# architsharma97/earl_benchmark

Measured on AMD Instinct MI355X. Metric: env steps/sec (aggregate) at N parallel envs, higher is better.
Workload: dtype f64

## Files before the change

### earl_benchmark_amd/csrc/tabletop_rollout_ws.h

```cpp
#pragma once
#include <type_traits>

#include "tabletop_device.h"

#ifndef EARL_WSM_OFF
#define EARL_WSM_OFF 0
#endif

#if !defined(EARL_WS_NO_SMALL_NT) && !defined(EARL_WS_SMALL_NT)
#define EARL_WS_SMALL_NT 1
#endif
#if !defined(EARL_WS_NO_XCD_REMAP) && !defined(EARL_WS_XCD_REMAP)
#define EARL_WS_XCD_REMAP 1
#endif
namespace earl {

typedef int ws_v4i __attribute__((ext_vector_type(4)));
typedef float ws_v4f __attribute__((ext_vector_type(4)));
__device__ __forceinline__ __amdgpu_buffer_rsrc_t ws_rsrc(const void* p) {
  return __builtin_amdgcn_make_buffer_rsrc(const_cast<void*>(p), 0, -1, 0x00020000);
}

struct WsArgs {
  int32_t n, T, horizon, wide;
  const float* __restrict__ act;
  double* __restrict__ qpos;
  int8_t* __restrict__ attached;
  const int32_t* __restrict__ goal_idx;
  const double* __restrict__ goal_table;
  int32_t* __restrict__ steps_since_reset;
  float* __restrict__ obs;
  float* __restrict__ reward;
  uint8_t* __restrict__ done;
  uint8_t* __restrict__ success;
  Thresholds th;
  float grip_x;
  int32_t reset_first;
  earl_tabletop_cfg cfg;
  int32_t* __restrict__ goal_idx_w;
  int32_t* __restrict__ num_interventions;
  int32_t episodes, Tep;
  long long act_ep_stride;
  int32_t wgs, ep_groups, ep_per_group;
};

__device__ __forceinline__ uint64_t ws_ep_counter(const WsArgs& a, int ep) { return a.cfg.counter + (uint64_t)ep * (uint64_t)(a.Tep + 1); }
__device__ __forceinline__ int ws_goal_row_ep(const WsArgs& a, int env, int ep) {
  if (a.reset_first) return sample_goal(a.cfg, ws_ep_counter(a, ep), env, nullptr);
  return a.goal_idx[env];
}

__device__ __forceinline__ int ws_goal_row(const WsArgs& a, int env) {
  if (a.reset_first) return sample_goal(a.cfg, a.cfg.counter, env, nullptr);
  return a.goal_idx[env];
}

__device__ __forceinline__ void wave_lds_fence() {
  __builtin_amdgcn_fence(__ATOMIC_RELEASE, "wavefront");
  __builtin_amdgcn_wave_barrier();
  __builtin_amdgcn_fence(__ATOMIC_ACQUIRE, "wavefront");
}

__device__ __forceinline__ double clip_fast(double x) { return fmin(fmax(x, -2.8), 2.8); }

template <bool EXACT>
__device__ __forceinline__ void ws_step(double& fx, double& fy, double& ox, double& oy, double& oxl, double& oyl,
                                        bool& att, double a0, double a1, bool grip, const Thresholds& th) {
  if constexpr (EXACT) {
    const double dx = fx - ox, dy = fy - oy;
    const bool near = fma(dy, dy, dx * dx) < th.grasp_d2;
    att = grip && (att || near);
    const double nfx = clipd(fx + a0, -2.8, 2.8), nfy = clipd(fy + a1, -2.8, 2.8);
    if (att) {
      ox = clipd(ox + (nfx - fx), -2.8, 2.8);
      oy = clipd(oy + (nfy - fy), -2.8, 2.8);
    }
    fx = nfx;
    fy = nfy;
    oxl = ox;
    oyl = oy;
  } else {
    const double dx = fx - oxl, dy = fy - oyl;
    const bool near = fma(dy, dy, dx * dx) < th.grasp_d2;
    att = grip && (att || near);
    oxl = ox;
    oyl = oy;
    const double nfx = clip_fast(fx + a0), nfy = clip_fast(fy + a1);
    const double ddx = att ? nfx - fx : -0.0, ddy = att ? nfy - fy : -0.0;
    ox = clip_fast(ox + ddx);
    oy = clip_fast(oy + ddy);
    fx = nfx;
    fy = nfy;
  }
}

struct WsConst { double lo, hi, thr; int nz; };
__device__ __forceinline__ void ws_step_v(double& fx, double& fy, double& ox, double& oy, double& oxl, double& oyl,
                                          int& att, double a0, double a1, int grip, const WsConst& k) {
  const double dx = fx - oxl, dy = fy - oyl;
  const int near = __double2hiint(fma(dy, dy, dx * dx) - k.thr) >> 31;
  att = grip & (att | near);
  oxl = ox;
  oyl = oy;
  const double nfx = fmin(fmax(fx + a0, k.lo), k.hi), nfy = fmin(fmax(fy + a1, k.lo), k.hi);
  const double ddx = nfx - fx, ddy = nfy - fy;
  const double sx = __hiloint2double((att & __double2hiint(ddx)) | (~att & k.nz), att & __double2loint(ddx));
  const double sy = __hiloint2double((att & __double2hiint(ddy)) | (~att & k.nz), att & __double2loint(ddy));
  ox = fmin(fmax(ox + sx, k.lo), k.hi);
  oy = fmin(fmax(oy + sy, k.lo), k.hi);
  fx = nfx;
  fy = nfy;
}

__device__ __forceinline__ double both_halves_from_lower(double v) {
  const unsigned lo = __double2loint(v), hi = __double2hiint(v);
  const auto r0 = __builtin_amdgcn_permlane32_swap(lo, lo, false, false);
  const auto r1 = __builtin_amdgcn_permlane32_swap(hi, hi, false, false);
  return __hiloint2double(r1[0], r0[0]);
}
template <bool EXACT>
__device__ __forceinline__ void ws_step_xy(double& f, double& o, double& ol, unsigned long long& att64, double a,
                                           unsigned long long grip64, const Thresholds& th) {
  const double d = f - (EXACT ? o : ol);
  const double d2 = fma(d, d, both_halves_from_lower(d * d));
  const unsigned near_y = (unsigned)(__ballot(d2 < th.grasp_d2) >> 32);
  const unsigned long long near64 = ((unsigned long long)near_y << 32) | near_y;
  att64 = grip64 & (att64 | near64);
  const bool att = __builtin_amdgcn_inverse_ballot_w64(att64);
  if constexpr (EXACT) {
    const double nf = clipd(f + a, -2.8, 2.8);
    if (att) o = clipd(o + (nf - f), -2.8, 2.8);
    f = nf;
    ol = o;
  } else {
    ol = o;
    const double nf = clip_fast(f + a);
    const double dd = att ? nf - f : -0.0;
    o = clip_fast(o + dd);
    f = nf;
  }
}

__device__ __forceinline__ unsigned long long ws_near_mask_xy(double f, double o, const Thresholds& th) {
  const double d = f - o;
  const double d2 = fma(d, d, both_halves_from_lower(d * d));
  const unsigned near_y = (unsigned)(__ballot(d2 < th.grasp_d2) >> 32);
  return ((unsigned long long)near_y << 32) | near_y;
}
__device__ __forceinline__ void ws_step_xy_pipe(double& f, double& o, unsigned long long& nm, unsigned long long& att64,
                                                double a, unsigned long long grip64, const Thresholds& th) {
  att64 = grip64 & (att64 | nm);
  const bool att = __builtin_amdgcn_inverse_ballot_w64(att64);
  const double nf = clip_fast(f + a);
  nm = ws_near_mask_xy(nf, o, th);
  const double dd = att ? nf - f : -0.0;
  o = clip_fast(o + dd);
  f = nf;
}

__device__ __forceinline__ double dpp_from_x(double v) {
  const int lo = __builtin_amdgcn_update_dpp(__double2loint(v), __double2loint(v), 0xA0, 0xF, 0xF, false);
  const int hi = __builtin_amdgcn_update_dpp(__double2hiint(v), __double2hiint(v), 0xA0, 0xF, 0xF, false);
  return __hiloint2double(hi, lo);
}
__device__ __forceinline__ double dpp_swap_pair(double v) {
  const int lo = __builtin_amdgcn_update_dpp(__double2loint(v), __double2loint(v), 0xB1, 0xF, 0xF, false);
  const int hi = __builtin_amdgcn_update_dpp(__double2hiint(v), __double2hiint(v), 0xB1, 0xF, 0xF, false);
  return __hiloint2double(hi, lo);
}
__device__ __forceinline__ int ws_near_mask_adj(double f, double o, const WsConst& k) {
  const double d = f - o;
  const double d2 = fma(d, d, dpp_from_x(d * d));
  const int m = __double2hiint(d2 - k.thr) >> 31;
  return __builtin_amdgcn_update_dpp(m, m, 0xF5, 0xF, 0xF, false);
}
__device__ __forceinline__ void ws_step_adj(double& f, double& o, int& nm, int& attm, double a, int grip, const WsConst& k) {
  attm = grip & (attm | nm);
  const double nf = fmin(fmax(f + a, k.lo), k.hi);
  nm = ws_near_mask_adj(nf, o, k);
  const double dd = nf - f;
  const double sd = __hiloint2double((attm & __double2hiint(dd)) | (~attm & k.nz), attm & __double2loint(dd));
  o = fmin(fmax(o + sd, k.lo), k.hi);
  f = nf;
}
__device__ __forceinline__ void ws_step_adj_exact(double& f, double& o, int& attm, double a, int grip, int c, const Thresholds& th) {
  const double pf = dpp_swap_pair(f), po = dpp_swap_pair(o), pa = dpp_swap_pair(a);
  double fx = c ? pf : f, fy = c ? f : pf, ox = c ? po : o, oy = c ? o : po, oxl = 0, oyl = 0;
  bool att = attm != 0;
  ws_step<true>(fx, fy, ox, oy, oxl, oyl, att, c ? pa : a, c ? a : pa, grip != 0, th);
  f = c ? fy : fx;
  o = c ? oy : ox;
  attm = att ? -1 : 0;
}

__device__ unsigned long long g_ws_prof[64 * 16];
__device__ __forceinline__ unsigned long long ws_clock() {
  unsigned long long t;
  asm volatile("s_memtime %0\n\ts_waitcnt lgkmcnt(0)" : "=s"(t)::"memory");
  return t;
}
#define WS_STAMP(acc)                                  \
  if constexpr (PROF) {                                \
    const unsigned long long t_ = ws_clock();          \
    acc += t_ - p_x;                                   \
    p_x = t_;                                          \
  }

template <int RT, int NC, int NL, int NS, int K, int LEAD, bool PROF = false, bool MULTI = false, bool LDNT = false>
__global__ __launch_bounds__(64 * ((NC == 3 ? 2 : NC) + NL + NS)) void rollout_ws_kernel(const WsArgs a_in) {
  constexpr int E = 64;
  WsArgs a = a_in;
#ifdef EARL_WS_XCD_REMAP
  const int bid = (gridDim.x % 8 == 0) ? (int)((blockIdx.x % 8) * (gridDim.x / 8) + blockIdx.x / 8) : (int)blockIdx.x;
#else
  const int bid = (int)blockIdx.x;
#endif
  int wg = bid;
  bool leaves_state = true;
  int eps_before = 0;
  if constexpr (MULTI) {
    if (a_in.ep_groups > 1) {
      const int grp = bid / a_in.wgs;
      wg = bid - grp * a_in.wgs;
      eps_before = grp * a_in.ep_per_group;
      const int ne = min(a_in.ep_per_group, a_in.episodes - eps_before);
      leaves_state = eps_before + ne == a_in.episodes;
      a.episodes = ne;
      a.T = ne * a_in.Tep;
      a.cfg.counter = a_in.cfg.counter + (uint64_t)eps_before * (uint64_t)(a_in.Tep + 1);
      const size_t row0 = (size_t)eps_before * (size_t)a_in.Tep * (size_t)a_in.n;
      a.act = a_in.act + (size_t)eps_before * (size_t)a_in.act_ep_stride;
      a.obs = a_in.obs + row0 * 12; a.reward = a_in.reward + row0; a.done = a_in.done + row0; a.success = a_in.success + row0;
    }
  }
  constexpr int NCW = NC == 3 ? 2 : NC;
  constexpr int KL = K / NL;
  static_assert(K % NL == 0, "K must be a multiple of NL");
  static_assert(!MULTI || NC == 3, "several episodes per launch: adjacent-lane compute waves only");
  static_assert(NC == 1 || NC == 2 || NC == 3, "NC is 1, 2 or 3");
  __shared__ double A[3][K][2 * E];
  __shared__ uint8_t G[3][K][E];
  __shared__ int slow_flag[3][NL];
  __shared__ float4 R[2][K][E * 3];
  constexpr int SQ = K >= 8 ? 1 : KL;
  __shared__ float S[NL][SQ][E * 3];

  const int wave = __builtin_amdgcn_readfirstlane(threadIdx.x >> 6), lane = threadIdx.x & 63;
  const int n = a.n, T = a.T;
  const int i0 = wg * E;
  const int i = i0 + lane;
  const int valid = min(E, n - i0);
  const bool live = lane < valid;
  const int nch = (T + K - 1) / K;
  unsigned long long p_x = 0, p_t0 = 0;

  if (wave < NCW || wave >= NCW + NL) {
    const int tid = wave < NCW ? (int)threadIdx.x : (int)threadIdx.x - 64 * NL;
    const int e = tid % E;
    float g[6] = {0, 0, 0, 0, 0, 0};
    if (e < valid) load_goal<1>(a.goal_table, ws_goal_row(a, i0 + e), g);
    for (int rowi = tid / E; rowi < 2 * K; rowi += NCW + NS) {
      float4* row = &R[0][0][0] + (size_t)rowi * (E * 3) + e * 3;
      row[1] = float4{-1.0f, -1.0f, g[0], g[1]};
      row[2] = float4{g[2], g[3], g[4], g[5]};
    }
  }

  if (wave < NCW) {
   __builtin_amdgcn_s_setprio(3);
   if constexpr (NC == 3) {
    const int h = lane & 1, el = lane >> 1, e = wave * 32 + el;
    const int ie = i0 + e;
    const bool alive = e < valid;
    double f = 0, o = 0;
    bool att0 = false;
    if (alive) {
      if (a.reset_first) {
        Env<1> ev;
        const int gi = reset_env<1>(ev, a.cfg, a.cfg.counter, ie, a.goal_table, nullptr, a.th);
        f = h ? ev.q[1] : ev.q[0];
        o = h ? ev.q[3] : ev.q[2];
        if (h == 0 && leaves_state) {
          a.goal_idx_w[ie] = gi;
          a.num_interventions[ie] += 1 + eps_before;
        }
      } else {
        f = a.qpos[(size_t)ie * 4 + h];
        o = a.qpos[(size_t)ie * 4 + 2 + h];
        att0 = a.attached[ie] >= 0;
      }
    }
    int attm = att0 ? -1 : 0;
    WsConst kc{-2.8, 2.8, a.th.grasp_d2, (int)0x80000000};
    asm volatile("" : "+v"(kc.lo), "+v"(kc.hi), "+v"(kc.thr), "+v"(kc.nz));
    int nm = ws_near_mask_adj(f, o, kc);
    bool slow = __any(!(fabs(f) <= 1e300) || !(fabs(o) <= 2.8));
    unsigned long long p_read = 0, p_comp = 0, p_bar = 0;
    if constexpr (PROF) p_t0 = ws_clock();
    __syncthreads();
    if constexpr (PROF) p_x = ws_clock();
    const unsigned long long p_first = p_x - p_t0;
    double av[K], nv[K];
    int gv[K], ng[K];
    int nslow = 0;
    auto fetch = [&](int c) {
      const int ab = c % 3;
      nslow = 0;
#pragma unroll
      for (int w = 0; w < NL; ++w) nslow |= slow_flag[ab][w];
#pragma unroll
      for (int k = 0; k < K; ++k) {
        nv[k] = A[ab][k][wave * 64 + lane];
        ng[k] = reinterpret_cast<const int8_t*>(&G[ab][k][0])[e];
      }
    };
    fetch(0);
    constexpr int GR = 8, GPC = K / GR;
    static_assert(!MULTI || (K % GR == 0 && GPC <= 2), "multi-episode launches: chunks of one or two 8-step granules");
    const int gpe = MULTI ? a.Tep / GR : 0x7fffffff;
    int next_ep_g = gpe, ep = 0, last_gi = -1;
    double f_pend = 0, o_pend = 0;
    bool pend = false;
    auto prepare_episode = [&](const int gidx) -> bool {
      if (MULTI && !(EARL_WSM_OFF & 4) && gidx == next_ep_g && gidx * GR < T) {
        ++ep;
        next_ep_g += gpe;
        Env<1> ev;
        last_gi = reset_env<1>(ev, a.cfg, ws_ep_counter(a, ep), ie, a.goal_table, nullptr, a.th);
        f_pend = h ? ev.q[1] : ev.q[0];
        o_pend = h ? ev.q[3] : ev.q[2];
        return true;
      }
      return false;
    };
    auto apply_episode = [&]() {
      f = f_pend; o = o_pend;
      attm = 0;
      nm = ws_near_mask_adj(f, o, kc);
    };
    for (int c = 0; c < nch; ++c) {
      const int rb = c & 1;
      if (prepare_episode(c * (MULTI ? GPC : 1))) apply_episode();
      if constexpr (MULTI && GPC == 2) pend = prepare_episode(c * GPC + 1);
      slow = slow || (nslow != 0);
#pragma unroll
      for (int k = 0; k < K; ++k) { av[k] = nv[k]; gv[k] = ng[k]; }
      if (c + 1 < nch) fetch(c + 1);
      if constexpr (PROF) asm volatile("s_waitcnt lgkmcnt(0)" ::: "memory");
      WS_STAMP(p_read)
      auto run = [&](auto exact, auto full) {
#pragma unroll
        for (int k = 0; k < K; ++k) {
          if constexpr (!decltype(full)::value)
            if (c * K + k >= T) break;
          if constexpr (MULTI && GPC == 2) { if (k == GR && pend) apply_episode(); }
          if constexpr (decltype(exact)::value) ws_step_adj_exact(f, o, attm, av[k], gv[k], h, a.th);
          else ws_step_adj(f, o, nm, attm, av[k], gv[k], kc);
          float* rowf = reinterpret_cast<float*>(&R[rb][k][e * 3]);
          rowf[h] = (float)f;
          rowf[2 + h] = (float)o;
          rowf[4 + h] = __int_as_float(~attm & (int)0xBF800000);
        }
      };
      const bool whole = (c + 1) * K <= T;
      if (__builtin_amdgcn_readfirstlane(slow ? 1 : 0)) {
        if (whole) run(std::true_type{}, std::true_type{}); else run(std::true_type{}, std::false_type{});
      } else {
        if (whole) run(std::false_type{}, std::true_type{}); else run(std::false_type{}, std::false_type{});
      }
      if constexpr (PROF) asm volatile("s_waitcnt lgkmcnt(0)" ::: "memory");
      WS_STAMP(p_comp)
      __syncthreads();
      WS_STAMP(p_bar)
    }
    if constexpr (PROF) {
      if (lane == 0 && bid < 64 && wave == 0) {
        unsigned long long* op = g_ws_prof + bid * 16;
        op[0] = p_first; op[1] = p_read; op[2] = p_comp; op[3] = p_bar; op[4] = p_x - p_t0;
      }
      if (lane == 0 && bid < 64 && wave == 1) g_ws_prof[bid * 16 + 13] = p_bar;
    }
    if (alive && leaves_state) {
      a.qpos[(size_t)ie * 4 + h] = f;
      a.qpos[(size_t)ie * 4 + 2 + h] = o;
      if (h == 0) {
        a.attached[ie] = attm ? 0 : -1;
        a.steps_since_reset[ie] = (a.reset_first ? 0 : a.steps_since_reset[ie]) + (MULTI ? a.Tep : T);
        if (MULTI && ep > 0) {
          a.goal_idx_w[ie] = last_gi;
          a.num_interventions[ie] += ep;
        }
      }
    }
   } else if constexpr (NC == 2) {
    const int h = lane >> 5, el = lane & 31, e = wave * 32 + el;
    const int ie = i0 + e;
    const bool alive = e < valid;
    double f = 0, o = 0;
    bool att0 = false;
    if (alive) {
      if (a.reset_first) {
        Env<1> ev;
        const int gi = reset_env<1>(ev, a.cfg, a.cfg.counter, ie, a.goal_table, nullptr, a.th);
        f = h ? ev.q[1] : ev.q[0];
        o = h ? ev.q[3] : ev.q[2];
        if (h == 0) {
          a.goal_idx_w[ie] = gi;
          a.num_interventions[ie] += 1;
        }
      } else {
        f = a.qpos[(size_t)ie * 4 + h];
        o = a.qpos[(size_t)ie * 4 + 2 + h];
        att0 = a.attached[ie] >= 0;
      }
    }
    double ol = o;
    unsigned long long att64 = __ballot(att0);
    unsigned long long nm = ws_near_mask_xy(f, o, a.th);
    bool slow = __any(!(fabs(f) <= 1e300) || !(fabs(o) <= 2.8));
    unsigned long long p_read = 0, p_comp = 0, p_bar = 0;
    if constexpr (PROF) p_t0 = ws_clock();
    __syncthreads();
    if constexpr (PROF) p_x = ws_clock();
    const unsigned long long p_first = p_x - p_t0;
    double av[K], nv[K];
    uint8_t gv[K], ng[K];
    int nslow = 0;
    auto fetch = [&](int c) {
      const int ab = c % 3;
      nslow = 0;
#pragma unroll
      for (int w = 0; w < NL; ++w) nslow |= slow_flag[ab][w];
#pragma unroll
      for (int k = 0; k < K; ++k) { nv[k] = A[ab][k][wave * 64 + lane]; ng[k] = G[ab][k][e]; }
    };
    fetch(0);
    for (int c = 0; c < nch; ++c) {
      const int rb = c & 1;
      slow = slow || (nslow != 0);
#pragma unroll
      for (int k = 0; k < K; ++k) { av[k] = nv[k]; gv[k] = ng[k]; }
      if (c + 1 < nch) fetch(c + 1);
      if constexpr (PROF) asm volatile("s_waitcnt lgkmcnt(0)" ::: "memory");
      WS_STAMP(p_read)
      auto run = [&](auto exact, auto full) {
#pragma unroll
        for (int k = 0; k < K; ++k) {
          if constexpr (!decltype(full)::value)
            if (c * K + k >= T) break;
          if constexpr (decltype(exact)::value) ws_step_xy<true>(f, o, ol, att64, av[k], __ballot(gv[k] != 0), a.th);
          else ws_step_xy_pipe(f, o, nm, att64, av[k], __ballot(gv[k] != 0), a.th);
          float* rowf = reinterpret_cast<float*>(&R[rb][k][e * 3]);
          rowf[h] = (float)f;
          rowf[2 + h] = (float)o;
          rowf[4 + h] = __builtin_amdgcn_inverse_ballot_w64(att64) ? 0.0f : -1.0f;
        }
      };
      const bool whole = (c + 1) * K <= T;
      if (__builtin_amdgcn_readfirstlane(slow ? 1 : 0)) {
        if (whole) run(std::true_type{}, std::true_type{}); else run(std::true_type{}, std::false_type{});
      } else {
        if (whole) run(std::false_type{}, std::true_type{}); else run(std::false_type{}, std::false_type{});
      }
      if constexpr (PROF) asm volatile("s_waitcnt lgkmcnt(0)" ::: "memory");
      WS_STAMP(p_comp)
      __syncthreads();
      WS_STAMP(p_bar)
    }
    if constexpr (PROF) {
      if (lane == 0 && bid < 64 && wave == 0) {
        unsigned long long* op = g_ws_prof + bid * 16;
        op[0] = p_first; op[1] = p_read; op[2] = p_comp; op[3] = p_bar; op[4] = p_x - p_t0;
      }
    }
    if (alive) {
      a.qpos[(size_t)ie * 4 + h] = f;
      a.qpos[(size_t)ie * 4 + 2 + h] = o;
      if (h == 0) {
        a.attached[ie] = (att64 >> lane) & 1 ? 0 : -1;
        a.steps_since_reset[ie] = (a.reset_first ? 0 : a.steps_since_reset[ie]) + T;
      }
    }
   } else {
    double fx = 0, fy = 0, ox = 0, oy = 0;
    bool att = false;
    if (live) {
      if (a.reset_first) {
        Env<1> ev;
        const int gi = reset_env<1>(ev, a.cfg, a.cfg.counter, i, a.goal_table, nullptr, a.th);
        fx = ev.q[0]; fy = ev.q[1]; ox = ev.q[2]; oy = ev.q[3];
        a.goal_idx_w[i] = gi;
        a.num_interventions[i] += 1;
      } else {
        const double2* q2 = reinterpret_cast<const double2*>(a.qpos + (size_t)i * 4);
        const double2 u = q2[0], v = q2[1];
        fx = u.x; fy = u.y; ox = v.x; oy = v.y;
        att = a.attached[i] >= 0;
      }
    }
    double oxl = ox, oyl = oy;
    int attm = att ? -1 : 0;
    WsConst kc{-2.8, 2.8, a.th.grasp_d2, (int)0x80000000};
    asm volatile("" : "+v"(kc.lo), "+v"(kc.hi), "+v"(kc.thr), "+v"(kc.nz));
    bool slow = __any(!(fabs(fx) <= 1e300) || !(fabs(fy) <= 1e300) || !(fabs(ox) <= 2.8) || !(fabs(oy) <= 2.8));
    unsigned long long p_read = 0, p_comp = 0, p_bar = 0;
    if constexpr (PROF) p_t0 = ws_clock();
    __syncthreads();
    if constexpr (PROF) p_x = ws_clock();
    const unsigned long long p_first = p_x - p_t0;
    double2 av[K], nv[K];
    int gv[K], ng[K];
    int nslow = 0;
    auto fetch = [&](int c) {
      const int ab = c % 3;
      nslow = 0;
#pragma unroll
      for (int w = 0; w < NL; ++w) nslow |= slow_flag[ab][w];
#pragma unroll
      for (int k = 0; k < K; ++k) {
        nv[k] = reinterpret_cast<const double2*>(&A[ab][k][0])[lane];
        ng[k] = reinterpret_cast<const int8_t*>(&G[ab][k][0])[lane];
      }
    };
    fetch(0);
    for (int c = 0; c < nch; ++c) {
      const int rb = c & 1;
      slow = slow || (nslow != 0);
#pragma unroll
      for (int k = 0; k < K; ++k) { av[k] = nv[k]; gv[k] = ng[k]; }
      if (c + 1 < nch) fetch(c + 1);
      if constexpr (PROF) asm volatile("s_waitcnt lgkmcnt(0)" ::: "memory");
      WS_STAMP(p_read)
      auto run = [&](auto exact, auto full) {
#pragma unroll
        for (int k = 0; k < K; ++k) {
          if constexpr (!decltype(full)::value)
            if (c * K + k >= T) break;
          if constexpr (decltype(exact)::value) {
            bool attb = attm != 0;
            ws_step<true>(fx, fy, ox, oy, oxl, oyl, attb, av[k].x, av[k].y, gv[k] != 0, a.th);
            attm = attb ? -1 : 0;
          } else {
            ws_step_v(fx, fy, ox, oy, oxl, oyl, attm, av[k].x, av[k].y, gv[k], kc);
          }
          float4* row = &R[rb][k][lane * 3];
          row[0] = float4{(float)fx, (float)fy, (float)ox, (float)oy};
          const float flag = __int_as_float(~attm & (int)0xBF800000);
          *reinterpret_cast<float2*>(&row[1]) = float2{flag, flag};
        }
      };
      const bool whole = (c + 1) * K <= T;
      if (__builtin_amdgcn_readfirstlane(slow ? 1 : 0)) {
        if (whole) run(std::true_type{}, std::true_type{}); else run(std::true_type{}, std::false_type{});
      } else {
        if (whole) run(std::false_type{}, std::true_type{}); else run(std::false_type{}, std::false_type{});
      }
      if constexpr (PROF) asm volatile("s_waitcnt lgkmcnt(0)" ::: "memory");
      WS_STAMP(p_comp)
      __syncthreads();
      WS_STAMP(p_bar)
    }
    if constexpr (PROF) {
      if (lane == 0 && bid < 64) {
        unsigned long long* o = g_ws_prof + bid * 16;
        o[0] = p_first; o[1] = p_read; o[2] = p_comp; o[3] = p_bar; o[4] = p_x - p_t0;
      }
    }
    if (live) {
      double2* q2 = reinterpret_cast<double2*>(a.qpos + (size_t)i * 4);
      q2[0] = double2{fx, fy};
      q2[1] = double2{ox, oy};
      a.attached[i] = attm ? 0 : -1;
      a.steps_since_reset[i] = (a.reset_first ? 0 : a.steps_since_reset[i]) + T;
    }
   }
  } else if (wave < NCW + NL) {
    const int w = wave - NCW;
    float rawA[LEAD][KL][3], rawB[LEAD][KL][3];
    const int last = max(valid * 3 - 1, 0);
    const int e0 = min(lane, last), e1 = min(lane + 64, last), e2 = min(lane + 128, last);
    const float* const base = a.act + (size_t)i0 * 3;
    const size_t step_stride = (size_t)n * 3;
    constexpr int GR = 8, GPC = MULTI ? K / GR : 1;
    const int gpe = MULTI ? a.Tep / GR : 0x7fffffff;
    int l_ep_end = gpe, l_ep_first = 0;
    size_t l_ep_base = 0;
    auto issue_trip = [&](float (&raw)[LEAD][KL][3], int r) {
      const float* rowp[LEAD][GPC];
      size_t off[LEAD][KL];
#pragma unroll
      for (int d = 0; d < LEAD; ++d) {
        if constexpr (MULTI && !(EARL_WSM_OFF & 1)) {
          const int j = min(r * LEAD + d, nch - 1);
#pragma unroll
          for (int hg = 0; hg < GPC; ++hg) {
            const int gidx = min(j * GPC + hg, T / GR - 1);
            const int xm = -(int)(gidx >= l_ep_end);
            l_ep_end += gpe & xm; l_ep_first += gpe & xm;
            l_ep_base += (size_t)a.act_ep_stride & (size_t)(long long)xm;
            rowp[d][hg] = base + l_ep_base + (size_t)__builtin_amdgcn_readfirstlane((gidx - l_ep_first) * GR + w) * step_stride;
          }
        } else {
#pragma unroll
          for (int q = 0; q < KL; ++q)
            off[d][q] = (size_t)__builtin_amdgcn_readfirstlane(min((r * LEAD + d) * K + q * NL + w, (MULTI ? a.Tep : T) - 1)) * step_stride;
        }
      }
      const size_t qstride = (size_t)NL * step_stride;
      static_assert(!MULTI || GR % NL == 0, "a loader's steps of a granule: a whole number");
      constexpr int QG = MULTI ? GR / NL : KL;
#pragma unroll
      for (int d = 0; d < LEAD; ++d) {
#pragma unroll
        for (int q = 0; q < KL; ++q) {
          const float* p;
          if constexpr (MULTI && !(EARL_WSM_OFF & 1)) p = rowp[d][q / QG] + (size_t)(q % QG) * qstride;
          else p = base + off[d][q];
#ifdef EARL_WS_LD_AUX
          if constexpr (true) {
            const __amdgpu_buffer_rsrc_t rs = ws_rsrc(p);
            raw[d][q][0] = __builtin_bit_cast(float, __builtin_amdgcn_raw_buffer_load_b32(rs, e0 * 4, 0, EARL_WS_LD_AUX));
            raw[d][q][1] = __builtin_bit_cast(float, __builtin_amdgcn_raw_buffer_load_b32(rs, e1 * 4, 0, EARL_WS_LD_AUX));
            raw[d][q][2] = __builtin_bit_cast(float, __builtin_amdgcn_raw_buffer_load_b32(rs, e2 * 4, 0, EARL_WS_LD_AUX));
          } else
#endif
          if constexpr (LDNT) {
            raw[d][q][0] = __builtin_nontemporal_load(p + e0); raw[d][q][1] = __builtin_nontemporal_load(p + e1); raw[d][q][2] = __builtin_nontemporal_load(p + e2);
          } else {
            raw[d][q][0] = p[e0]; raw[d][q][1] = p[e1]; raw[d][q][2] = p[e2];
          }
        }
      }
    };
    unsigned long long p_proc = 0, p_bar = 0;
    auto process = [&](const float (&raw)[KL][3], int j) {
      const int ab = j % 3;
      bool any_nan = false;
#pragma unroll
      for (int q0 = 0; q0 < KL; q0 += SQ) {
#pragma unroll
        for (int q = q0; q < q0 + SQ; ++q) {
          float* sk = &S[w][q - q0][0];
          sk[lane] = raw[q][0]; sk[lane + 64] = raw[q][1]; sk[lane + 128] = raw[q][2];
        }
        wave_lds_fence();
#pragma unroll
        for (int q = q0; q < q0 + SQ; ++q) {
          const float* sk = &S[w][q - q0][0];
          const float r0 = sk[lane * 3], r1 = sk[lane * 3 + 1], r2 = sk[lane * 3 + 2];
          const double a0 = rescale_action(r0), a1 = rescale_action(r1);
          any_nan = any_nan || (r0 != r0) || (r1 != r1);
          if (j < nch) {
            if constexpr (NC == 2) {
              A[ab][q * NL + w][(lane >> 5) * 64 + (lane & 31)] = a0;
              A[ab][q * NL + w][(lane >> 5) * 64 + 32 + (lane & 31)] = a1;
            } else {
              reinterpret_cast<double2*>(&A[ab][q * NL + w][0])[lane] = double2{a0, a1};
            }
            G[ab][q * NL + w][lane] = (uint8_t)(r2 >= a.grip_x ? 0xFF : 0);
          }
        }
        wave_lds_fence();
      }
      const bool wave_nan = __any(any_nan);
      if (lane == 0 && j < nch) slow_flag[ab][w] = wave_nan ? 1 : 0;
    };
    auto run_trip = [&](float (&cur)[LEAD][KL][3], float (&nxt)[LEAD][KL][3], int r) {
#pragma unroll
      for (int d = 0; d < LEAD; ++d) {
        const int j = r * LEAD + d;
        process(cur[d], j);
        if (d == 0) {
          __builtin_amdgcn_sched_barrier(0);
          issue_trip(nxt, r + 1);
          __builtin_amdgcn_sched_barrier(0);
        }
        WS_STAMP(p_proc)
        if (j >= 1 && j < nch + 2) __syncthreads();
        WS_STAMP(p_bar)
      }
    };
    if constexpr (PROF) p_t0 = p_x = ws_clock();
    issue_trip(rawA, 0);
    for (int r = 0; r * LEAD < nch + 2; r += 2) {
      run_trip(rawA, rawB, r);
      if ((r + 1) * LEAD < nch + 2) run_trip(rawB, rawA, r + 1);
    }
    if constexpr (PROF) {
      if (lane == 0 && bid < 64 && w == 0) {
        unsigned long long* o = g_ws_prof + bid * 16;
        o[5] = p_proc; o[6] = p_bar; o[7] = p_x - p_t0;
      }
      if (lane == 0 && bid < 64 && w == NL - 1 && NL > 1) {
        unsigned long long* o = g_ws_prof + bid * 16;
        o[14] = p_proc; o[15] = p_bar;
      }
    }
  } else {
    const int s = wave - NCW - NL;
    float g[6] = {0, 0, 0, 0, 0, 0};
    int t_done = 0x7fffffff;
    if (live) {
      load_goal<1>(a.goal_table, ws_goal_row(a, i), g);
      const long long td = (long long)a.horizon - 1 - (a.reset_first ? 0 : a.steps_since_reset[i]);
      t_done = td < 0 ? 0 : (td > 0x7fffffff ? 0x7fffffff : (int)td);
    }
    constexpr int GR = 8, GPC = MULTI ? K / GR : 1;
    const int gpe = MULTI ? a.Tep / GR : 0x7fffffff;
    int g_ep = 0, t_ep0 = 0, g_end = gpe;
    float gn[6] = {0, 0, 0, 0, 0, 0};
    bool gn_stale = false;
    if (MULTI && live) load_goal<1>(a.goal_table, ws_goal_row_ep(a, i, 1), gn);
    auto reload_next_goal = [&]() {
      if (MULTI && gn_stale) {
        gn_stale = false;
        if (live) load_goal<1>(a.goal_table, ws_goal_row_ep(a, i, g_ep + 1), gn);
      }
    };
    auto enter_episode = [&](int gidx) {
      if (MULTI && !(EARL_WSM_OFF & 2) && gidx >= g_end) {
        g_ep += 1; g_end += gpe; t_ep0 += a.Tep;
#pragma unroll
        for (int k = 0; k < 6; ++k) g[k] = gn[k];
        gn_stale = true;
      }
    };
    auto refill_goal = [&](int gidx) {
      if (MULTI && !(EARL_WSM_OFF & 2) && g_end <= gidx + 2 * GPC && (gidx / GPC) + 2 < nch) {
        reload_next_goal();
        const int k0 = (gidx % GPC) * GR;
        for (int k = k0 + (s % GR); k < k0 + GR; k += NS) {
          if ((k % NS) != s) continue;
          float4* row = &R[(gidx / GPC) & 1][k][lane * 3];
          row[1] = float4{-1.0f, -1.0f, gn[0], gn[1]};
          row[2] = float4{gn[2], gn[3], gn[4], gn[5]};
        }
      }
    };
    asm volatile("s_waitcnt vmcnt(0)" ::: "memory");
    const bool full = (valid == E) && ((n & 3) == 0);
    unsigned long long p_st = 0, p_bar = 0;
    auto store_chunk = [&](int c) {
      const int rb = c & 1;
#pragma unroll
      for (int k = 0; k < K; ++k) {
        if constexpr (MULTI) {
          if (k % GR == 0) {
            if (k > 0) refill_goal(c * GPC + k / GR - 1);
            enter_episode(c * GPC + k / GR);
          }
        }
        if ((k % NS) != s) continue;
        const int t = c * K + k;
        if (t >= T) continue;
        const size_t row0 = (size_t)t * n + i0;
        float4* dst = reinterpret_cast<float4*>(a.obs + row0 * 12);
        const float4* src = &R[rb][k][0];
        const float4 p = src[lane * 3];
        const float o[12] = {p.x, p.y, p.z, p.w, 0.f, 0.f, g[0], g[1], g[2], g[3], g[4], g[5]};
        const bool succ = success1(o, a.wide, a.th);
        float rew;
        if constexpr (RT == EARL_REWARD_SPARSE) rew = succ ? 1.0f : 0.0f;
        else rew = (float)dense1(o);
        const bool dn = t - t_ep0 >= t_done;
        if (full) {
          const float4 v0 = src[lane], v1 = src[lane + 64], v2 = src[lane + 128];
          dst[lane] = v0; dst[lane + 64] = v1; dst[lane + 128] = v2;
          a.reward[row0 + lane] = rew;
          const unsigned long long ms = __ballot(succ), md = __ballot(dn);
          if (lane < 16) {
            const uint32_t ns = (uint32_t)(ms >> (4 * lane)) & 0xFu, nd = (uint32_t)(md >> (4 * lane)) & 0xFu;
            reinterpret_cast<uint32_t*>(a.success + row0)[lane] = (ns * 0x00204081u) & 0x01010101u;
            reinterpret_cast<uint32_t*>(a.done + row0)[lane] = (nd * 0x00204081u) & 0x01010101u;
          }
        } else {
#pragma unroll
          for (int m = 0; m < 3; ++m) {
            const int idx = lane + 64 * m;
            if (idx < valid * 3) dst[idx] = src[idx];
          }
          if (live) {
            a.reward[row0 + lane] = rew;
            a.success[row0 + lane] = succ;
            a.done[row0 + lane] = dn;
          }
        }
      }
      if constexpr (MULTI) refill_goal(c * GPC + GPC - 1);
    };
    constexpr int Q = (K % NS == 0) ? K / NS : 0;
    auto store_chunk_fast = [&](int c) {
      const int rb = c & 1;
      struct Rows { float4 v0, v1, v2, p; };
      auto load_rows = [&](const int q) -> Rows {
        const float4* src = &R[rb][s + NS * q][0];
        return Rows{src[lane], src[lane + 64], src[lane + 128], src[lane * 3]};
      };
      const Rows r0 = load_rows(0), r1 = load_rows(Q > 1 ? 1 : 0), r2 = load_rows(Q > 2 ? 2 : 0), r3 = load_rows(Q > 3 ? 3 : 0);
      auto step_q = [&](auto qc, const Rows rw) __attribute__((always_inline)) {
        constexpr int q = decltype(qc)::value;
        if constexpr (MULTI) enter_episode(c * GPC + q);
        const int t = c * K + s + NS * q;
        const size_t row0 = (size_t)t * n + i0;
        float4* dst = reinterpret_cast<float4*>(a.obs + row0 * 12);
#ifdef EARL_WS_NO_STORES
        if ((t & 63) == 0) { dst[lane] = rw.v0; dst[lane + 64] = rw.v1; dst[lane + 128] = rw.v2; }
#elif defined(EARL_WS_ST_AUX)
        {
          const __amdgpu_buffer_rsrc_t rs = ws_rsrc(dst);
          __builtin_amdgcn_raw_buffer_store_b128(__builtin_bit_cast(ws_v4i, ws_v4f{rw.v0.x, rw.v0.y, rw.v0.z, rw.v0.w}), rs, lane * 16, 0, EARL_WS_ST_AUX);
          __builtin_amdgcn_raw_buffer_store_b128(__builtin_bit_cast(ws_v4i, ws_v4f{rw.v1.x, rw.v1.y, rw.v1.z, rw.v1.w}), rs, (lane + 64) * 16, 0, EARL_WS_ST_AUX);
          __builtin_amdgcn_raw_buffer_store_b128(__builtin_bit_cast(ws_v4i, ws_v4f{rw.v2.x, rw.v2.y, rw.v2.z, rw.v2.w}), rs, (lane + 128) * 16, 0, EARL_WS_ST_AUX);
        }
#elif !defined(EARL_WS_TEMPORAL_STORES)
        typedef float nt4 __attribute__((ext_vector_type(4)));
        nt4* d4 = reinterpret_cast<nt4*>(dst);
        __builtin_nontemporal_store(nt4{rw.v0.x, rw.v0.y, rw.v0.z, rw.v0.w}, d4 + lane);
        __builtin_nontemporal_store(nt4{rw.v1.x, rw.v1.y, rw.v1.z, rw.v1.w}, d4 + lane + 64);
        __builtin_nontemporal_store(nt4{rw.v2.x, rw.v2.y, rw.v2.z, rw.v2.w}, d4 + lane + 128);
#else
        dst[lane] = rw.v0; dst[lane + 64] = rw.v1; dst[lane + 128] = rw.v2;
#endif
        const float o[12] = {rw.p.x, rw.p.y, rw.p.z, rw.p.w, 0.f, 0.f, g[0], g[1], g[2], g[3], g[4], g[5]};
        const bool succ = success1(o, a.wide, a.th);
        float rew;
        if constexpr (RT == EARL_REWARD_SPARSE) rew = succ ? 1.0f : 0.0f;
        else rew = (float)dense1(o);
#ifdef EARL_WS_NO_STORES
        if ((t & 63) == 0) a.reward[row0 + lane] = rew;
#elif defined(EARL_WS_SMALL_NT)
        __builtin_nontemporal_store(rew, a.reward + row0 + lane);
#else
        a.reward[row0 + lane] = rew;
#endif
        const unsigned long long ms = __ballot(succ), md = __ballot(t - t_ep0 >= t_done);
#ifdef EARL_WS_NO_STORES
        if (lane < 16 && (t & 63) == 0) {
#else
        if (lane < 16) {
#endif
          const uint32_t ns = (uint32_t)(ms >> (4 * lane)) & 0xFu, nd = (uint32_t)(md >> (4 * lane)) & 0xFu;
#ifdef EARL_WS_SMALL_NT
          __builtin_nontemporal_store((ns * 0x00204081u) & 0x01010101u, reinterpret_cast<uint32_t*>(a.success + row0) + lane);
          __builtin_nontemporal_store((nd * 0x00204081u) & 0x01010101u, reinterpret_cast<uint32_t*>(a.done + row0) + lane);
#else
          reinterpret_cast<uint32_t*>(a.success + row0)[lane] = (ns * 0x00204081u) & 0x01010101u;
          reinterpret_cast<uint32_t*>(a.done + row0)[lane] = (nd * 0x00204081u) & 0x01010101u;
#endif
        }
        if constexpr (MULTI) refill_goal(c * GPC + q);
      };
      static_assert(Q <= 4, "steps of a chunk per storer");
      if constexpr (Q > 0) step_q(std::integral_constant<int, 0>{}, r0);
      if constexpr (Q > 1) step_q(std::integral_constant<int, 1>{}, r1);
      if constexpr (Q > 2) step_q(std::integral_constant<int, 2>{}, r2);
      if constexpr (Q > 3) step_q(std::integral_constant<int, 3>{}, r3);
    };
    auto store = [&](int c) {
      reload_next_goal();
      if (Q > 0 && (!MULTI || NS == GR) && full && (c + 1) * K <= T) store_chunk_fast(c);
      else store_chunk(c);
    };
    if constexpr (PROF) p_t0 = ws_clock();
    __syncthreads();
    if constexpr (PROF) p_x = ws_clock();
    for (int c = 0; c < nch; ++c) {
      if (c >= 1) store(c - 1);
      WS_STAMP(p_st)
      __syncthreads();
      WS_STAMP(p_bar)
    }
    store(nch - 1);
    if constexpr (PROF) {
      if (lane == 0 && bid < 64 && s == 0) {
        unsigned long long* o = g_ws_prof + bid * 16;
        o[8] = p_st; o[9] = p_bar; o[10] = ws_clock() - p_t0;
      }
      if (lane == 0 && bid == 0 && gridDim.x <= 32) {
        unsigned long long* o = g_ws_prof + (32 + s) * 16;
        o[8] = p_st; o[9] = p_bar;
      }
      if (lane == 0 && bid < 64 && s == NS - 1 && NS > 1) {
        unsigned long long* o = g_ws_prof + bid * 16;
        o[11] = p_st; o[12] = p_bar;
      }
    }
  }
}
#undef WS_STAMP

}
```

Before: 76.71 billion.

## Pack compute-wave step records compactly and rebuild observation rows in storer registers

For the adjacent-lane compute layout, compute waves now write only position floats plus a per-chunk bitmask of attachment flags, instead of full 12-float observation rows with goal values. Grip commands are likewise packed into one bitmask word per env rather than a byte per step. Storer waves rebuild each observation row in registers from the packed records, per-lane goal values and lane masks, which removes the goal refill writes to shared memory. The compute loop is unrolled by two so the record buffer index is a compile-time immediate. This cuts shared-memory traffic and LDS footprint on the compute critical path, at the cost of extra ALU work and register pressure in the storers.

Result: no change. 76.85 billion, median of 6 (+0.2%).

```diff
diff --git a/earl_benchmark_amd/csrc/tabletop_rollout_ws.h b/earl_benchmark_amd/csrc/tabletop_rollout_ws.h
--- a/earl_benchmark_amd/csrc/tabletop_rollout_ws.h
+++ b/earl_benchmark_amd/csrc/tabletop_rollout_ws.h
@@ -239,10 +239,14 @@
   static_assert(!MULTI || NC == 3, "several episodes per launch: adjacent-lane compute waves only");
   static_assert(NC == 1 || NC == 2 || NC == 3, "NC is 1, 2 or 3");
   __shared__ double A[3][K][2 * E];
-  __shared__ uint8_t G[3][K][E];
+  constexpr bool REC = NC == 3;
+  static_assert(!REC || K <= 16, "records: the step's LDS offsets are instruction immediates (2 K steps of 4 units < 256); grip and flag bits fit a word");
+  __shared__ uint32_t FLW[2][REC ? 2 * E : 1];
+  __shared__ uint8_t G[3][REC ? 1 : K][E];
+  __shared__ uint32_t GW[3][NL][REC ? E : 1];
   __shared__ int slow_flag[3][NL];
-  __shared__ float4 R[2][K][E * 3];
-  constexpr int SQ = K >= 8 ? 1 : KL;
+  __shared__ float4 R[2][K][REC ? E : E * 3];
+  constexpr int SQ = REC ? KL : (K >= 8 ? 1 : KL);
   __shared__ float S[NL][SQ][E * 3];
 
   const int wave = __builtin_amdgcn_readfirstlane(threadIdx.x >> 6), lane = threadIdx.x & 63;
@@ -254,7 +258,7 @@
   const int nch = (T + K - 1) / K;
   unsigned long long p_x = 0, p_t0 = 0;
 
-  if (wave < NCW || wave >= NCW + NL) {
+  if (!REC && (wave < NCW || wave >= NCW + NL)) {
     const int tid = wave < NCW ? (int)threadIdx.x : (int)threadIdx.x - 64 * NL;
     const int e = tid % E;
     float g[6] = {0, 0, 0, 0, 0, 0};
@@ -300,21 +304,20 @@
     __syncthreads();
     if constexpr (PROF) p_x = ws_clock();
     const unsigned long long p_first = p_x - p_t0;
-    double av[K], nv[K];
-    int gv[K], ng[K];
+    double av0[K], av1[K];
+    int gw0 = 0, gw1 = 0;
     int nslow = 0;
-    auto fetch = [&](int c) {
+    auto fetch = [&](int c, double (&nv)[K], int& ngw) {
       const int ab = c % 3;
       nslow = 0;
-#pragma unroll
-      for (int w = 0; w < NL; ++w) nslow |= slow_flag[ab][w];
-#pragma unroll
-      for (int k = 0; k < K; ++k) {
-        nv[k] = A[ab][k][wave * 64 + lane];
-        ng[k] = reinterpret_cast<const int8_t*>(&G[ab][k][0])[e];
-      }
-    };
-    fetch(0);
+      ngw = 0;
+#pragma unroll
+      for (int w = 0; w < NL; ++w) { nslow |= slow_flag[ab][w]; ngw |= (int)GW[ab][w][e]; }
+#pragma unroll
+      for (int k = 0; k < K; ++k) nv[k] = A[ab][k][wave * 64 + lane];
+    };
+    fetch(0, av0, gw0);
+    float* const rec = reinterpret_cast<float*>(&R[0][0][0]) + wave * 64 + lane;
     constexpr int GR = 8, GPC = K / GR;
     static_assert(!MULTI || (K % GR == 0 && GPC <= 2), "multi-episode launches: chunks of one or two 8-step granules");
     const int gpe = MULTI ? a.Tep / GR : 0x7fffffff;
@@ -338,28 +341,27 @@
       attm = 0;
       nm = ws_near_mask_adj(f, o, kc);
     };
-    for (int c = 0; c < nch; ++c) {
-      const int rb = c & 1;
+    auto chunk = [&](const int c, auto rbc, const double (&av)[K], const int gw, double (&nv)[K], int& ngw) {
+      constexpr int RB = decltype(rbc)::value;
       if (prepare_episode(c * (MULTI ? GPC : 1))) apply_episode();
       if constexpr (MULTI && GPC == 2) pend = prepare_episode(c * GPC + 1);
       slow = slow || (nslow != 0);
-#pragma unroll
-      for (int k = 0; k < K; ++k) { av[k] = nv[k]; gv[k] = ng[k]; }
-      if (c + 1 < nch) fetch(c + 1);
+      if (c + 1 < nch) fetch(c + 1, nv, ngw);
       if constexpr (PROF) asm volatile("s_waitcnt lgkmcnt(0)" ::: "memory");
       WS_STAMP(p_read)
+      unsigned fb = 0;
       auto run = [&](auto exact, auto full) {
 #pragma unroll
         for (int k = 0; k < K; ++k) {
           if constexpr (!decltype(full)::value)
-            if (c * K + k >= T) break;
+            if (c * K + k >= T) { fb >>= K - k; break; }
           if constexpr (MULTI && GPC == 2) { if (k == GR && pend) apply_episode(); }
-          if constexpr (decltype(exact)::value) ws_step_adj_exact(f, o, attm, av[k], gv[k], h, a.th);
-          else ws_step_adj(f, o, nm, attm, av[k], gv[k], kc);
-          float* rowf = reinterpret_cast<float*>(&R[rb][k][e * 3]);
-          rowf[h] = (float)f;
-          rowf[2 + h] = (float)o;
-          rowf[4 + h] = __int_as_float(~attm & (int)0xBF800000);
+          const int grip = (int)((unsigned)gw << (31 - k)) >> 31;
+          if constexpr (decltype(exact)::value) ws_step_adj_exact(f, o, attm, av[k], grip, h, a.th);
+          else ws_step_adj(f, o, nm, attm, av[k], grip, kc);
+          rec[(RB * K + k) * (E * 4)] = (float)f;
+          rec[(RB * K + k) * (E * 4) + 2 * E] = (float)o;
+          fb = __builtin_amdgcn_alignbit((unsigned)attm, fb, 1);
         }
       };
       const bool whole = (c + 1) * K <= T;
@@ -368,10 +370,15 @@
       } else {
         if (whole) run(std::false_type{}, std::true_type{}); else run(std::false_type{}, std::false_type{});
       }
+      FLW[RB][wave * 64 + lane] = fb;
       if constexpr (PROF) asm volatile("s_waitcnt lgkmcnt(0)" ::: "memory");
       WS_STAMP(p_comp)
       __syncthreads();
       WS_STAMP(p_bar)
+    };
+    for (int c = 0; c < nch; c += 2) {
+      chunk(c, std::integral_constant<int, 0>{}, av0, gw0, av1, gw1);
+      if (c + 1 < nch) chunk(c + 1, std::integral_constant<int, 1>{}, av1, gw1, av0, gw0);
     }
     if constexpr (PROF) {
       if (lane == 0 && bid < 64 && wave == 0) {
@@ -636,6 +643,7 @@
     auto process = [&](const float (&raw)[KL][3], int j) {
       const int ab = j % 3;
       bool any_nan = false;
+      [[maybe_unused]] uint32_t gbits = 0;
 #pragma unroll
       for (int q0 = 0; q0 < KL; q0 += SQ) {
 #pragma unroll
@@ -657,11 +665,15 @@
             } else {
               reinterpret_cast<double2*>(&A[ab][q * NL + w][0])[lane] = double2{a0, a1};
             }
-            G[ab][q * NL + w][lane] = (uint8_t)(r2 >= a.grip_x ? 0xFF : 0);
+            const bool grip = r2 >= a.grip_x;
+            if constexpr (REC) gbits |= (grip ? 1u : 0u) << (q * NL + w);
+            else G[ab][q * NL + w][lane] = (uint8_t)(grip ? 0xFF : 0);
           }
         }
         wave_lds_fence();
       }
+      if constexpr (REC)
+        if (j < nch) GW[ab][w][lane] = gbits;
       const bool wave_nan = __any(any_nan);
       if (lane == 0 && j < nch) slow_flag[ab][w] = wave_nan ? 1 : 0;
     };
@@ -698,10 +710,35 @@
     }
   } else {
     const int s = wave - NCW - NL;
-    float g[6] = {0, 0, 0, 0, 0, 0};
+    const int rj = lane % 3, mp0 = (3 - rj) % 3;
+    const int e0 = (lane + 64 * mp0) / 3, e1 = (lane + 64 * ((mp0 + 1) % 3)) / 3, e2 = (lane + 64 * ((mp0 + 2) % 3)) / 3;
+    int m0[3], m1[3];
+#pragma unroll
+    for (int m = 0; m < 3; ++m) {
+      m0[m] = (rj + m) % 3 == 0 ? -1 : 0;
+      m1[m] = (rj + m) % 3 == 1 ? -1 : 0;
+      if constexpr (REC) asm volatile("" : "+v"(m0[m]), "+v"(m1[m]));
+    }
+    float g[6] = {0, 0, 0, 0, 0, 0}, gr[12] = {0, 0, 0, 0, 0, 0, 0, 0, 0, 0, 0, 0};
+    auto load_goals = [&](const int ep, float (&go)[6], float (&gro)[12]) {
+      if (live) load_goal<1>(a.goal_table, ws_goal_row_ep(a, i, ep), go);
+      if constexpr (REC) {
+        float t1[6] = {0, 0, 0, 0, 0, 0}, t2[6] = {0, 0, 0, 0, 0, 0};
+        if (e1 < valid) load_goal<1>(a.goal_table, ws_goal_row_ep(a, i0 + e1, ep), t1);
+        if (e2 < valid) load_goal<1>(a.goal_table, ws_goal_row_ep(a, i0 + e2, ep), t2);
+#pragma unroll
+        for (int m = 0; m < 3; ++m) {
+          const int part = (rj + m) % 3;
+          gro[4 * m + 0] = part == 2 ? t2[2] : 0.f;
+          gro[4 * m + 1] = part == 2 ? t2[3] : 0.f;
+          gro[4 * m + 2] = part == 2 ? t2[4] : part == 1 ? t1[0] : 0.f;
+          gro[4 * m + 3] = part == 2 ? t2[5] : part == 1 ? t1[1] : 0.f;
+        }
+      }
+    };
+    load_goals(0, g, gr);
     int t_done = 0x7fffffff;
     if (live) {
-      load_goal<1>(a.goal_table, ws_goal_row(a, i), g);
       const long long td = (long long)a.horizon - 1 - (a.reset_first ? 0 : a.steps_since_reset[i]);
       t_done = td < 0 ? 0 : (td > 0x7fffffff ? 0x7fffffff : (int)td);
     }
@@ -709,12 +746,13 @@
     const int gpe = MULTI ? a.Tep / GR : 0x7fffffff;
     int g_ep = 0, t_ep0 = 0, g_end = gpe;
     float gn[6] = {0, 0, 0, 0, 0, 0};
+    float grn[12] = {0, 0, 0, 0, 0, 0, 0, 0, 0, 0, 0, 0};
     bool gn_stale = false;
-    if (MULTI && live) load_goal<1>(a.goal_table, ws_goal_row_ep(a, i, 1), gn);
+    if constexpr (MULTI) load_goals(1, gn, grn);
     auto reload_next_goal = [&]() {
       if (MULTI && gn_stale) {
         gn_stale = false;
-        if (live) load_goal<1>(a.goal_table, ws_goal_row_ep(a, i, g_ep + 1), gn);
+        load_goals(g_ep + 1, gn, grn);
       }
     };
     auto enter_episode = [&](int gidx) {
@@ -722,19 +760,35 @@
         g_ep += 1; g_end += gpe; t_ep0 += a.Tep;
 #pragma unroll
         for (int k = 0; k < 6; ++k) g[k] = gn[k];
+#pragma unroll
+        for (int k = 0; k < 12; ++k) gr[k] = grn[k];
         gn_stale = true;
       }
     };
-    auto refill_goal = [&](int gidx) {
-      if (MULTI && !(EARL_WSM_OFF & 2) && g_end <= gidx + 2 * GPC && (gidx / GPC) + 2 < nch) {
-        reload_next_goal();
-        const int k0 = (gidx % GPC) * GR;
-        for (int k = k0 + (s % GR); k < k0 + GR; k += NS) {
-          if ((k % NS) != s) continue;
-          float4* row = &R[(gidx / GPC) & 1][k][lane * 3];
-          row[1] = float4{-1.0f, -1.0f, gn[0], gn[1]};
-          row[2] = float4{gn[2], gn[3], gn[4], gn[5]};
-        }
+    static_assert(!MULTI || REC, "several episodes per launch: the goal part of the rows comes from the storers' registers");
+    struct Rows { float4 v0, v1, v2, p; };
+    auto load_rows = [&](const int rb, const int k) -> Rows {
+      const float4* src = &R[rb][k][0];
+      if constexpr (REC) {
+        const float2* pl = reinterpret_cast<const float2*>(src);
+        const float2 f0 = pl[e0], o0 = pl[E + e0], fp = pl[lane], op = pl[E + lane];
+        const int att = (int)(FLW[rb][2 * e1] << (K - 1 - k)) >> 31;
+        const float fl = __int_as_float(~att & (int)0xBF800000);
+        return Rows{float4{f0.x, f0.y, o0.x, o0.y}, float4{fl, fl, 0.f, 0.f}, float4{0.f, 0.f, 0.f, 0.f}, float4{fp.x, fp.y, op.x, op.y}};
+      } else {
+        return Rows{src[lane], src[lane + 64], src[lane + 128], src[lane * 3]};
+      }
+    };
+    auto form_rows = [&](const Rows r) -> Rows {
+      if constexpr (REC) {
+        const int x = __float_as_int(r.v0.x), y = __float_as_int(r.v0.y), z = __float_as_int(r.v0.z), w = __float_as_int(r.v0.w), fl = __float_as_int(r.v1.x);
+        auto part = [&](const int m) {
+          return float4{__int_as_float(__float_as_int(gr[4 * m + 0]) | (x & m0[m]) | (fl & m1[m])), __int_as_float(__float_as_int(gr[4 * m + 1]) | (y & m0[m]) | (fl & m1[m])),
+                        __int_as_float(__float_as_int(gr[4 * m + 2]) | (z & m0[m])), __int_as_float(__float_as_int(gr[4 * m + 3]) | (w & m0[m]))};
+        };
+        return Rows{part(0), part(1), part(2), r.p};
+      } else {
+        return r;
       }
     };
     asm volatile("s_waitcnt vmcnt(0)" ::: "memory");
@@ -745,18 +799,15 @@
 #pragma unroll
       for (int k = 0; k < K; ++k) {
         if constexpr (MULTI) {
-          if (k % GR == 0) {
-            if (k > 0) refill_goal(c * GPC + k / GR - 1);
-            enter_episode(c * GPC + k / GR);
-          }
+          if (k % GR == 0) enter_episode(c * GPC + k / GR);
         }
         if ((k % NS) != s) continue;
         const int t = c * K + k;
         if (t >= T) continue;
         const size_t row0 = (size_t)t * n + i0;
         float4* dst = reinterpret_cast<float4*>(a.obs + row0 * 12);
-        const float4* src = &R[rb][k][0];
-        const float4 p = src[lane * 3];
+        const Rows rw = form_rows(load_rows(rb, k));
+        const float4 p = rw.p;
         const float o[12] = {p.x, p.y, p.z, p.w, 0.f, 0.f, g[0], g[1], g[2], g[3], g[4], g[5]};
         const bool succ = success1(o, a.wide, a.th);
         float rew;
@@ -764,8 +815,7 @@
         else rew = (float)dense1(o);
         const bool dn = t - t_ep0 >= t_done;
         if (full) {
-          const float4 v0 = src[lane], v1 = src[lane + 64], v2 = src[lane + 128];
-          dst[lane] = v0; dst[lane + 64] = v1; dst[lane + 128] = v2;
+          dst[lane] = rw.v0; dst[lane + 64] = rw.v1; dst[lane + 128] = rw.v2;
           a.reward[row0 + lane] = rew;
           const unsigned long long ms = __ballot(succ), md = __ballot(dn);
           if (lane < 16) {
@@ -774,11 +824,9 @@
             reinterpret_cast<uint32_t*>(a.done + row0)[lane] = (nd * 0x00204081u) & 0x01010101u;
           }
         } else {
-#pragma unroll
-          for (int m = 0; m < 3; ++m) {
-            const int idx = lane + 64 * m;
-            if (idx < valid * 3) dst[idx] = src[idx];
-          }
+          if (lane < valid * 3) dst[lane] = rw.v0;
+          if (lane + 64 < valid * 3) dst[lane + 64] = rw.v1;
+          if (lane + 128 < valid * 3) dst[lane + 128] = rw.v2;
           if (live) {
             a.reward[row0 + lane] = rew;
             a.success[row0 + lane] = succ;
@@ -786,20 +834,16 @@
           }
         }
       }
-      if constexpr (MULTI) refill_goal(c * GPC + GPC - 1);
     };
     constexpr int Q = (K % NS == 0) ? K / NS : 0;
     auto store_chunk_fast = [&](int c) {
       const int rb = c & 1;
-      struct Rows { float4 v0, v1, v2, p; };
-      auto load_rows = [&](const int q) -> Rows {
-        const float4* src = &R[rb][s + NS * q][0];
-        return Rows{src[lane], src[lane + 64], src[lane + 128], src[lane * 3]};
-      };
-      const Rows r0 = load_rows(0), r1 = load_rows(Q > 1 ? 1 : 0), r2 = load_rows(Q > 2 ? 2 : 0), r3 = load_rows(Q > 3 ? 3 : 0);
-      auto step_q = [&](auto qc, const Rows rw) __attribute__((always_inline)) {
+      const Rows r0 = load_rows(rb, s), r1 = load_rows(rb, s + NS * (Q > 1 ? 1 : 0)), r2 = load_rows(rb, s + NS * (Q > 2 ? 2 : 0)),
+                 r3 = load_rows(rb, s + NS * (Q > 3 ? 3 : 0));
+      auto step_q = [&](auto qc, const Rows rl) __attribute__((always_inline)) {
         constexpr int q = decltype(qc)::value;
         if constexpr (MULTI) enter_episode(c * GPC + q);
+        const Rows rw = form_rows(rl);
         const int t = c * K + s + NS * q;
         const size_t row0 = (size_t)t * n + i0;
         float4* dst = reinterpret_cast<float4*>(a.obs + row0 * 12);
@@ -848,7 +892,6 @@
           reinterpret_cast<uint32_t*>(a.done + row0)[lane] = (nd * 0x00204081u) & 0x01010101u;
 #endif
         }
-        if constexpr (MULTI) refill_goal(c * GPC + q);
       };
       static_assert(Q <= 4, "steps of a chunk per storer");
       if constexpr (Q > 0) step_q(std::integral_constant<int, 0>{}, r0);
```
